# theEricMa/ScaleDreamer

Hardware: AMD Instinct MI355X
Metric: ASD train steps/sec (64x64 render, SD2.1) (higher is better)
Workload: dtype f32 renderer / f16 diffusion (f32 accumulate); 1 GPU; asd_sd_nerf: 1 view/GPU, 64x64 rays, 512 spp occgrid march, implicit-volume iNGP (16x2 hash grid 2^19, MLP 64), SD-2.1 UNet batch 5 (CFG+Perp-Neg+shifted t), VAE 512^2 fwd+bwd, AdamW; views_per_gpu=1, parallelism=dp1, diffusion_backend=hip, diffusion_weights=seeded random init (seed 1)

## Files before the change

include/asd_hip.h:

```cpp
#ifndef ASD_HIP_H
#define ASD_HIP_H

#include <stdint.h>

#ifdef __cplusplus
extern "C" {
#endif

#define ASD_MAX_LEVELS 16
#define ASD_OK 0
#define ASD_ERR_ARG 1
#define ASD_ERR_LAUNCH 2
#define ASD_ERR_UNSUPPORTED 3

typedef struct asd_grid_meta {
    uint32_t n_levels;
    uint32_t n_features;
    uint32_t n_params;
    uint32_t reserved;
    float    scale[ASD_MAX_LEVELS];
    uint32_t resolution[ASD_MAX_LEVELS];
    uint32_t offset[ASD_MAX_LEVELS];
    uint32_t size[ASD_MAX_LEVELS];
    uint32_t dense[ASD_MAX_LEVELS];
// ... 252 lines not shown
    int32_t gn_silu;
    int32_t wide_rows;
    int32_t ln_mode;
    float   ln_eps;
    const float* ln_sc;
    float*  ln_stats;
    int32_t a_seg_rows, w_seg_rows;
    int32_t a_seg_off[9], w_seg_off[6];
    int32_t partials_only;
    int32_t gn_apply;
    void*   gn_apply_y;
    const void* gn_apply_gamma; const void* gn_apply_beta;
    float   gn_apply_eps;
    int32_t gn_apply_silu;
    float*  gn_apply_stats;
} asd_gemm_args;
int32_t asd_gemm_gn_records(const asd_gemm_args* args);
int32_t asd_gemm_gn_applies(const asd_gemm_args* args);
int asd_gemm_f16(const asd_gemm_args* args, void* stream);
int asd_gemm_force_tile(int32_t cfg);
enum { ASD_TILE_PLAIN = 0, ASD_TILE_WIN = 1, ASD_TILE_WIN2 = 2, ASD_TILE_PP = 3, ASD_TILE_WS = 4 };
int asd_gemm_tile_info(int32_t i, int32_t* out7);

#define ASD_GN_STATS_FLOATS(batch) (64 * (batch) + 64 * (512 + (batch)))
int asd_groupnorm_f16(const void* x1, int32_t c1, const void* x2, int32_t c2, int32_t batch, int32_t hw,
                      const void* gamma, const void* beta, float eps, int32_t silu, void* y,
                      float* stats ,
                      void* stream);
int asd_groupnorm_ordered_f16(const void* x, int32_t c, int32_t batch, int32_t hw, const void* gamma, const void* beta, float eps,
                              int32_t silu, void* y, float* stats, void* stream);
// ... 280 lines not shown
```

scaledreamer_amd/_lib.py:

```python
from __future__ import annotations

import ctypes as C
import os
from typing import Optional

import torch

_HERE = os.path.dirname(os.path.abspath(__file__))
LIB_PATH = os.environ.get("ASD_HIP_LIB") or os.path.join(_HERE, "libasd_hip.so")
ASD_MAX_LEVELS = 16

ASD_BIAS_CONST, ASD_BIAS_BLOB_MAGIC3D, ASD_BIAS_BLOB_DREAMFUSION, ASD_BIAS_SPHERE = 0, 1, 2, 3
ASD_FIELD_DENSITY, ASD_FIELD_SDF = 0, 1
ASD_ACT_SOFTPLUS, ASD_ACT_EXP, ASD_ACT_TRUNC_EXP, ASD_ACT_NONE = 0, 1, 2, 3


class AsdError(RuntimeError):
    pass


class GridMeta(C.Structure):
    _fields_ = [
        ("n_levels", C.c_uint32),
        ("n_features", C.c_uint32),
# ... 42 lines not shown
        ("lda", C.c_int32), ("ldw", C.c_int32), ("ldc", C.c_int32),
        ("bias", C.c_void_p), ("row_bias", C.c_void_p), ("rows_per_group", C.c_int32),
        ("residual", C.c_void_p), ("ldr", C.c_int32), ("act", C.c_int32), ("out_f32", C.c_int32),
        ("conv", C.c_int32), ("Hin", C.c_int32), ("Win", C.c_int32), ("Cin", C.c_int32), ("Hout", C.c_int32),
        ("Wout", C.c_int32), ("stride", C.c_int32), ("pad", C.c_int32), ("upsample", C.c_int32),
        ("zero_page", C.c_void_p), ("split_k", C.c_int32), ("workspace", C.c_void_p),
        ("tile_cfg", C.c_int32), ("ld_row_bias", C.c_int32), ("group_m", C.c_int32), ("group_n", C.c_int32),
        ("gn_partials", C.c_void_p), ("gn_cg", C.c_int32), ("gn_rows", C.c_int32),
        ("gn_bwd_x", C.c_void_p), ("gn_bwd_fstats", C.c_void_p), ("gn_bwd_gamma", C.c_void_p), ("gn_bwd_beta", C.c_void_p),
        ("gn_eps", C.c_float), ("gn_silu", C.c_int32), ("wide_rows", C.c_int32),
        ("ln_mode", C.c_int32), ("ln_eps", C.c_float), ("ln_sc", C.c_void_p), ("ln_stats", C.c_void_p),
        ("a_seg_rows", C.c_int32), ("w_seg_rows", C.c_int32), ("a_seg_off", C.c_int32 * 9), ("w_seg_off", C.c_int32 * 6),
        ("partials_only", C.c_int32),
        ("gn_apply", C.c_int32), ("gn_apply_y", C.c_void_p), ("gn_apply_gamma", C.c_void_p), ("gn_apply_beta", C.c_void_p),
        ("gn_apply_eps", C.c_float), ("gn_apply_silu", C.c_int32), ("gn_apply_stats", C.c_void_p),
    ]


class RenderParams(C.Structure):
    _fields_ = [("march", MarchCfg), ("meta", C.c_void_p), ("field", C.c_void_p), ("rays_o", C.c_void_p), ("rays_d", C.c_void_p), ("n_rays", C.c_int32),
                ("occ_bits", C.c_void_p), ("jitter", C.c_void_p), ("grid", C.c_void_p), ("w1d", C.c_void_p), ("w2d", C.c_void_p), ("w1f", C.c_void_p),
                ("w2f", C.c_void_p), ("bg", C.c_void_p), ("early_stop_eps", C.c_float), ("alpha_thre", C.c_float), ("prune", C.c_int32),
                ("color_act", C.c_int32), ("capacity", C.c_int32)]


RENDER_LAYOUT_FIELDS = ["total_bytes", "count", "offset", "total", "c_ray_idx", "c_t0", "c_t1", "c_pts", "c_sigma", "keep", "kept", "koff", "n_kept",
                        "ray_idx", "t0", "t1", "pts", "dirs", "sigma", "feats", "enc", "weights", "opacity", "depth", "z_var", "rgb_fg", "comp_rgb",
                        "c_feats", "c_enc"]


# ... 173 lines not shown
```

scaledreamer_amd/csrc/gemm_ws.hip:

```cpp
#include <type_traits>

#include "gemm_tile.h"

typedef float floatx16 __attribute__((ext_vector_type(16)));
typedef unsigned uintx4 __attribute__((ext_vector_type(4)));

#define WS_A_BYTES(NB) ((NB) * 64 * 64)
#define WS_W_BYTES (9 * 64 * 64)
#define WS_PAD 1024
#define WS_LDS_BYTES(NB) (3 * WS_W_BYTES + 2 * WS_A_BYTES(NB) + 2 * WS_PAD)

template <int NB>
__global__ __launch_bounds__(256, 1) void conv3x3_ws_kernel(const asd_gemm_args p) {
    constexpr int A_BYTES = WS_A_BYTES(NB), W_BYTES = WS_W_BYTES;
    constexpr int A_INSTR = A_BYTES / 1024;
    constexpr int A_PER_WAVE = (A_INSTR + 1) / 2;
    extern __shared__ __attribute__((aligned(16))) char smem[];
    char* const w_base = smem;
    char* const a_base = smem + 3 * W_BYTES + WS_PAD;
    const int tid = threadIdx.x, lane = tid & 63, wave = __builtin_amdgcn_readfirstlane(tid >> 6);
    const int wm = wave >> 1, wn = wave & 1;
    const int tiles_n = p.N / 64;
    const int tn = (int)blockIdx.x % tiles_n, kz = (int)blockIdx.x / tiles_n;
    const int n0 = tn * 64;
    const int cs = p.Cin / p.split_k, c0 = kz * cs, n_chunks = cs / 32;
    const bool w_loader = wave < 2;

    const int a_px = lane >> 2;
    const char* a_lane = (const char*)p.A + ((size_t)a_px * p.Cin + c0) * 2;
    const int a_piece_even = ((lane & 3) ^ (a_px >> 3)) * 16, a_piece_odd = ((lane & 3) ^ (2 + (a_px >> 3))) * 16;
    const char* w_lane = (const char*)p.W + ((size_t)(n0 + (lane >> 2)) * p.ldw + c0) * 2 + (((lane & 3) ^ ((lane >> 4) & 3)) * 16);

    auto issue_w = [&](int chunk) {
        char* W_s = w_base + (chunk % 3) * W_BYTES;
#pragma unroll
        for (int j = 0; j < 18; ++j) {
            const int t = wave * 18 + j;
            const size_t off = ((size_t)((t & 3) * 16) * p.ldw + (size_t)(t >> 2) * p.Cin + chunk * 32) * 2;
            __builtin_amdgcn_global_load_lds((const GLOBAL_AS void*)(w_lane + off), (LDS_AS void*)(W_s + t * 1024), 16, 0, 0);
        }
    };
    auto issue_a = [&](int chunk) {
        char* A_s = a_base + (chunk & 1) * A_BYTES;
#pragma unroll
        for (int j = 0; j < A_PER_WAVE; ++j) {
            const int q = (wave - 2) * A_PER_WAVE + j;
            if (q < A_INSTR)
                __builtin_amdgcn_global_load_lds((const GLOBAL_AS void*)(a_lane + ((size_t)q * 16 * p.Cin + chunk * 32) * 2 + ((q & 1) ? a_piece_odd : a_piece_even)),
                                                 (LDS_AS void*)(A_s + q * 1024), 16, 0, 0);
        }
    };

    const int l31 = lane & 31, kh = lane >> 5, yy = l31 >> 3, xx = l31 & 7;
    const unsigned m_x_first = xx == 0 ? 0u : 0xffffffffu, m_x_last = xx == 7 ? 0u : 0xffffffffu;
    const unsigned m_y_first = yy == 0 ? 0u : 0xffffffffu, m_y_last = yy == 3 ? 0u : 0xffffffffu;
    const bool top0 = ((wm * NB) & 1) == 0, top1 = ((wm * NB + 1) & 1) == 0;
    const unsigned m_ky0[2] = {top0 ? m_y_first : 0xffffffffu, top1 ? m_y_first : 0xffffffffu};
    const unsigned m_ky2[2] = {top0 ? 0xffffffffu : m_y_last, top1 ? 0xffffffffu : m_y_last};
    const unsigned a_lane_lds = (unsigned)(size_t)a_base + (unsigned)((wm * NB * 32 + yy * 8 + xx - 9) * 64);
    const unsigned w_lane_lds = (unsigned)(size_t)w_base + (unsigned)((wn * 32 + l31) * 64);
    const int wkey = (l31 >> 2) & 3;
    unsigned a_piece[3][2], w_piece[2];
#pragma unroll
    for (int j = 0; j < 2; ++j) {
        w_piece[j] = (unsigned)(((2 * j + kh) ^ wkey) * 16);
#pragma unroll
        for (int ky = 0; ky < 3; ++ky) a_piece[ky][j] = (unsigned)((((2 * j + kh) ^ ((yy + ky - 1) & 3))) * 16);
    }

    floatx16 acc[NB];
#pragma unroll
    for (int i = 0; i < NB; ++i)
#pragma unroll
        for (int r = 0; r < 16; ++r) acc[i][r] = 0.f;

    struct Frag { uintx4 a[NB]; uintx4 w; };
#define WS_READ16(dst, addr, OFF) asm volatile("ds_read_b128 %0, %1 offset:%2" : "=&v"(dst) : "v"(addr), "n"(OFF) : "memory")

    if (w_loader) {
        issue_w(0);
        if (n_chunks > 1) { issue_w(1); asm volatile("s_waitcnt vmcnt(18)" ::: "memory"); }
        else asm volatile("s_waitcnt vmcnt(0)" ::: "memory");
    } else {
        issue_a(0);
        asm volatile("s_waitcnt vmcnt(0)" ::: "memory");
    }
    __builtin_amdgcn_s_barrier();
    for (int c = 0; c < n_chunks; ++c) {
        if (w_loader) { if (c + 2 < n_chunks) issue_w(c + 2); }
        else if (c + 1 < n_chunks) issue_a(c + 1);
        const unsigned a_slot = a_lane_lds + (unsigned)((c & 1) * A_BYTES), w_slot = w_lane_lds + (unsigned)((c % 3) * W_BYTES);
        unsigned aaddr[3][2], waddr[2];
#pragma unroll
        for (int j = 0; j < 2; ++j) {
            waddr[j] = w_slot + w_piece[j];
#pragma unroll
            for (int ky = 0; ky < 3; ++ky) aaddr[ky][j] = a_slot + a_piece[ky][j];
        }
        auto read_frags = [&](Frag& f, auto step_c) {
            constexpr int step = decltype(step_c)::value, tap = step >> 1, j = step & 1, ky = tap / 3, kx = tap - ky * 3;
            WS_READ16(f.w, waddr[j], tap * 4096);
#define WS_RA(I_) if constexpr (I_ < NB) WS_READ16(f.a[I_], aaddr[ky][j], I_ * 2048 + (8 * ky + kx) * 64)
            WS_RA(0); WS_RA(1); WS_RA(2); WS_RA(3); WS_RA(4);
#undef WS_RA
        };
        auto mma = [&](Frag& f, auto step_c) {
            constexpr int step = decltype(step_c)::value, tap = step >> 1, ky = tap / 3, kx = tap - ky * 3;
            const unsigned mx = kx == 0 ? m_x_first : (kx == 2 ? m_x_last : 0xffffffffu);
            const unsigned m0 = mx & (ky == 0 ? m_ky0[0] : (ky == 2 ? m_ky2[0] : 0xffffffffu));
            const unsigned m1 = mx & (ky == 0 ? m_ky0[1] : (ky == 2 ? m_ky2[1] : 0xffffffffu));
#pragma unroll
            for (int i = 0; i < NB; ++i) {
                if (tap != 4) {
                    const unsigned m = (i & 1) ? m1 : m0;
                    f.a[i][0] &= m; f.a[i][1] &= m; f.a[i][2] &= m; f.a[i][3] &= m;
                }
                acc[i] = __builtin_amdgcn_mfma_f32_32x32x16_f16(__builtin_bit_cast(half8, f.a[i]), __builtin_bit_cast(half8, f.w), acc[i], 0, 0, 0);
            }
        };
        auto wait_frags = [&](Frag& f, auto pending_c) {
            constexpr int pending = decltype(pending_c)::value;
            if constexpr (NB == 5) asm volatile("s_waitcnt lgkmcnt(%6)" : "+v"(f.a[0]), "+v"(f.a[1]), "+v"(f.a[2]), "+v"(f.a[3]), "+v"(f.a[4]), "+v"(f.w) : "n"(pending));
            else if constexpr (NB == 4) asm volatile("s_waitcnt lgkmcnt(%5)" : "+v"(f.a[0]), "+v"(f.a[1]), "+v"(f.a[2]), "+v"(f.a[3]), "+v"(f.w) : "n"(pending));
            else if constexpr (NB == 3) asm volatile("s_waitcnt lgkmcnt(%4)" : "+v"(f.a[0]), "+v"(f.a[1]), "+v"(f.a[2]), "+v"(f.w) : "n"(pending));
            else if constexpr (NB == 2) asm volatile("s_waitcnt lgkmcnt(%3)" : "+v"(f.a[0]), "+v"(f.a[1]), "+v"(f.w) : "n"(pending));
            else asm volatile("s_waitcnt lgkmcnt(%2)" : "+v"(f.a[0]), "+v"(f.w) : "n"(pending));
        };
        Frag f0, f1;
        read_frags(f0, std::integral_constant<int, 0>{});
#define WS_STEP(S_, CUR_, NXT_)                                                                                   \
        if constexpr (S_ + 1 < 18) {                                                                              \
            read_frags(NXT_, std::integral_constant<int, (S_ + 1 < 18 ? S_ + 1 : 17)>{});                          \
            wait_frags(CUR_, std::integral_constant<int, NB + 1>{});                                              \
        } else wait_frags(CUR_, std::integral_constant<int, 0>{});                                                \
        mma(CUR_, std::integral_constant<int, S_>{});                                                             \
        __builtin_amdgcn_sched_barrier(0)
        WS_STEP(0, f0, f1); WS_STEP(1, f1, f0); WS_STEP(2, f0, f1); WS_STEP(3, f1, f0); WS_STEP(4, f0, f1); WS_STEP(5, f1, f0);
        WS_STEP(6, f0, f1); WS_STEP(7, f1, f0); WS_STEP(8, f0, f1); WS_STEP(9, f1, f0); WS_STEP(10, f0, f1); WS_STEP(11, f1, f0);
        WS_STEP(12, f0, f1); WS_STEP(13, f1, f0); WS_STEP(14, f0, f1); WS_STEP(15, f1, f0); WS_STEP(16, f0, f1); WS_STEP(17, f1, f0);
#undef WS_STEP
        if (w_loader && c + 2 < n_chunks) asm volatile("s_waitcnt vmcnt(18)" ::: "memory");
        else asm volatile("s_waitcnt vmcnt(0)" ::: "memory");
        __builtin_amdgcn_s_barrier();
    }
#undef WS_READ16

    float* slab = p.workspace + (size_t)kz * p.M * p.N + n0 + wn * 32 + l31;
#pragma unroll
    for (int i = 0; i < NB; ++i) {
        const int mt = wm * NB + i;
#pragma unroll
        for (int q = 0; q < 4; ++q)
#pragma unroll
            for (int r = 0; r < 4; ++r) {
                const int m = mt * 32 + q * 8 + kh * 4 + r;
                slab[(size_t)m * p.N] = acc[i][q * 4 + r];
            }
    }
}

size_t asd_conv_ws_lds_bytes(int images) { return (size_t)WS_LDS_BYTES(images); }

int asd_conv_ws_launch(const asd_gemm_args* a, hipStream_t s) {
    const int images = a->M / 64;
    const dim3 grid((a->N / 64) * a->split_k);
#define WS_LAUNCH(NB_) asd_launch_lds<conv3x3_ws_kernel<NB_>>(grid, dim3(256), asd_conv_ws_lds_bytes(NB_), s, *a)
    switch (images) {
        case 1: WS_LAUNCH(1); break;
        case 2: WS_LAUNCH(2); break;
        case 3: WS_LAUNCH(3); break;
        case 4: WS_LAUNCH(4); break;
        case 5: WS_LAUNCH(5); break;
        default: return ASD_ERR_ARG;
    }
#undef WS_LAUNCH
    return ASD_OK;
}
```

scaledreamer_amd/csrc/net.hip:

```cpp
#include <cstdlib>
#include <map>
#include <string>
#include <vector>

#include "asd_common.h"

namespace {

typedef _Float16 half_t;

struct WSpec { std::string name; int rows, cols; };

struct Bump {
    char* base = nullptr;
    size_t off = 0, cap = 0;
    void* take(size_t bytes) {
        off = (off + 255) & ~(size_t)255;
        void* p = base ? base + off : nullptr;
        off += bytes;
        return p;
    }
    half_t* halfs(size_t n) { return (half_t*)take(n * 2); }
    float* floats(size_t n) { return (float*)take(n * 4); }
};
// ... 38 lines not shown
        return (int)specs.size() - 1;
    }
    const half_t* w(const std::string& name) const {
        auto it = index.find(name);
        return it == index.end() ? nullptr : (const half_t*)ptr[it->second];
    }
    bool has(const std::string& name) const { return index.count(name) != 0; }
};

int pad32(int c) { return (c + 31) / 32 * 32; }

struct GemmOpt {
    const void* bias = nullptr; const void* row_bias = nullptr; int rows_per_group = 1, ld_row_bias = 0;
    const void* residual = nullptr; int ldr = 0; int act = 0; int out_f32 = 0;
    int gn_rows = 0;
    Act* out = nullptr;
    const half_t* gn_x = nullptr; const float* gn_fstats = nullptr; const half_t* gn_gamma = nullptr; const half_t* gn_beta = nullptr;
    int gn_silu = 0;
    bool gn_bwd_form = false;
    int ln_mode = 0; const float* ln_sc = nullptr; float* ln_stats = nullptr;
    const GnNext* gn_next = nullptr;
};

void set_gn_bwd(asd_gemm_args& g, const GemmOpt& o) {
    g.gn_bwd_x = o.gn_x; g.gn_bwd_fstats = o.gn_fstats; g.gn_bwd_gamma = o.gn_gamma; g.gn_bwd_beta = o.gn_beta;
    g.gn_eps = 1e-6f; g.gn_silu = o.gn_silu;
}

void launch_gemm(Run& r, asd_gemm_args& g, Act* gn_out = nullptr, bool gn_bwd_form = false, const GnNext* gn_next = nullptr) {
    g.zero_page = r.zero_page;
// ... 53 lines not shown
    g.ln_mode = o.ln_mode; g.ln_sc = o.ln_sc; g.ln_stats = o.ln_stats; g.ln_eps = 1e-5f;
    if (o.gn_x) set_gn_bwd(g, o);
    if (o.out) { *o.out = Act{}; o.out->p = (const half_t*)C; }
    launch_gemm(r, g, o.out, o.gn_bwd_form, o.gn_next);
}

void conv3x3(Run& r, const void* x, int B, int Hin, int Win, int Cin, const void* W, int Cout, void* y, int Hout, int Wout, int stride,
             int pad, int upsample, const GemmOpt& o = GemmOpt()) {
    asd_gemm_args g = asd_gemm_args{};
    const int taps = upsample == 3 ? 4 : 9;
    g.A = x; g.W = W; g.C = y; g.M = B * Hout * Wout; g.N = Cout; g.K = taps * Cin; g.lda = 0; g.ldw = taps * Cin; g.ldc = Cout;
    g.bias = o.bias; g.row_bias = o.row_bias; g.rows_per_group = o.row_bias ? o.rows_per_group : 1; g.ld_row_bias = o.ld_row_bias;
    g.residual = o.residual; g.ldr = o.ldr; g.act = o.act; g.out_f32 = o.out_f32;
    g.conv = 1; g.Hin = Hin; g.Win = Win; g.Cin = Cin; g.Hout = Hout; g.Wout = Wout; g.stride = stride; g.pad = pad; g.upsample = upsample;
    g.gn_rows = o.gn_rows;
    if (o.gn_x) set_gn_bwd(g, o);
    if (o.out) { *o.out = Act{}; o.out->p = (const half_t*)y; }
    launch_gemm(r, g, o.out, o.gn_bwd_form, o.gn_next);
}

#define LEAF(call)                                              \
    do {                                                        \
        if (!r.dry && r.status == ASD_OK) {                     \
            const int st__ = (call);                            \
            if (st__ != ASD_OK) r.status = st__;                \
        }                                                       \
    } while (0)

half_t* groupnorm(Run& r, const void* x1, int c1, const void* x2, int c2, int B, int hw, const half_t* gamma, const half_t* beta, float eps,
                  int silu, half_t* y = nullptr, float** stats_out = nullptr, const Act* src = nullptr) {
// ... 14 lines not shown
struct UBlock { std::vector<ULayer> layers; };

struct UNet : Net {
    asd_unet_desc d;
    std::vector<UBlock> inputs, outputs;
    UBlock middle;
    std::map<std::string, int> emb_off, ctx_off;
    int emb_total = 0, ctx_total = 0;
};

#define ASD_LN_FOLD_MIN_C 1024
void u_norm(UNet& n, const std::string& p, int c) { n.add(p + ".weight", 1, c); n.add(p + ".bias", 1, c); }
void u_lin(UNet& n, const std::string& p, int cin, int cout, bool bias = true) { n.add(p + ".weight", cout, cin); if (bias) n.add(p + ".bias", 1, cout); }
void u_conv(UNet& n, const std::string& p, int cin, int cout) { n.add(p + ".weight", cout, 9 * pad32(cin)); n.add(p + ".bias", 1, cout); }

void u_res(UNet& n, const std::string& p, int cin, int cout) {
    u_norm(n, p + ".in_layers.0", cin);
    u_conv(n, p + ".in_layers.2", cin, cout);
    u_norm(n, p + ".out_layers.0", cout);
    u_conv(n, p + ".out_layers.3", cout, cout);
    if (cin != cout) u_lin(n, p + ".skip_connection", cin, cout);
    n.emb_off[p] = n.emb_total;
    n.emb_total += cout;
}
void u_attn(UNet& n, const std::string& p, int c) {
    u_norm(n, p + ".norm", c);
    u_lin(n, p + ".proj_in", c, c);
    for (int dd = 0; dd < n.d.transformer_depth; ++dd) {
        const std::string b = p + ".transformer_blocks." + std::to_string(dd);
        const bool fold = c >= ASD_LN_FOLD_MIN_C;
        if (!fold) for (const char* nm : {".norm1", ".norm2", ".norm3"}) u_norm(n, b + nm, c);
        n.add(b + ".attn1.to_qk.weight", 2 * c, c);
        if (fold) n.add(b + ".attn1.to_qk.ln_sc", 1, 4 * 2 * c);
        n.add(b + ".attn1.to_v.weight", c, c);
        if (fold) n.add(b + ".attn1.to_v.ln_sc", 1, 4 * c);
// ... 13 lines not shown
void unet_build(UNet& n) {
    const asd_unet_desc& d = n.d;
    const int mc = d.model_channels, emb = 4 * mc;
    u_lin(n, "time_embed.0", mc, emb);
    u_lin(n, "time_embed.2", emb, emb);
    if (d.camera_dim > 0) { u_lin(n, "camera_embed.0", d.camera_dim, emb); u_lin(n, "camera_embed.2", emb, emb); }
    u_conv(n, "input_blocks.0.0", d.in_channels, mc);
    n.inputs.push_back(UBlock{{ULayer{0, "input_blocks.0.0", d.in_channels, mc}}});
    std::vector<int> chans{mc};
    int ch = mc, ds = 0;
    for (int lvl = 0; lvl < d.n_levels; ++lvl) {
        const int mult = d.channel_mult[lvl];
        for (int k = 0; k < d.num_res_blocks; ++k) {
            const std::string p = "input_blocks." + std::to_string(n.inputs.size());
            UBlock b;
            u_res(n, p + ".0", ch, mult * mc);
            b.layers.push_back(ULayer{1, p + ".0", ch, mult * mc});
            ch = mult * mc;
            if (d.attention_ds_mask & (1 << ds)) { u_attn(n, p + ".1", ch); b.layers.push_back(ULayer{2, p + ".1", ch, ch}); }
            n.inputs.push_back(b);
            chans.push_back(ch);
        }
        if (lvl != d.n_levels - 1) {
            const std::string p = "input_blocks." + std::to_string(n.inputs.size()) + ".0.op";
            u_conv(n, p, ch, ch);
            n.inputs.push_back(UBlock{{ULayer{3, p, ch, ch}}});
            chans.push_back(ch);
            ++ds;
        }
    }
    u_res(n, "middle_block.0", ch, ch);
    u_attn(n, "middle_block.1", ch);
    u_res(n, "middle_block.2", ch, ch);
    n.middle.layers = {ULayer{1, "middle_block.0", ch, ch}, ULayer{2, "middle_block.1", ch, ch}, ULayer{1, "middle_block.2", ch, ch}};
    for (int lvl = d.n_levels - 1; lvl >= 0; --lvl) {
        const int mult = d.channel_mult[lvl];
        for (int i = 0; i <= d.num_res_blocks; ++i) {
            const int ich = chans.back();
            chans.pop_back();
            const std::string p = "output_blocks." + std::to_string(n.outputs.size());
            UBlock b;
            u_res(n, p + ".0", ch + ich, mc * mult);
            b.layers.push_back(ULayer{1, p + ".0", ch + ich, mc * mult});
            ch = mc * mult;
            int k = 1;
            if (d.attention_ds_mask & (1 << ds)) {
                u_attn(n, p + "." + std::to_string(k), ch);
                b.layers.push_back(ULayer{2, p + "." + std::to_string(k), ch, ch});
                ++k;
            }
            if (lvl && i == d.num_res_blocks) {
                const std::string q = p + "." + std::to_string(k) + ".conv";
                n.add(q + ".weight", 4 * ch, 4 * pad32(ch)); n.add(q + ".bias", 1, ch);
                b.layers.push_back(ULayer{4, q, ch, ch});
                --ds;
            }
            n.outputs.push_back(b);
// ... 21 lines not shown
    return dst;
}

Act u_resblock(UNet& n, Run& r, const UState& s, const std::string& p, const Act& xin, int cin, int cout, int Hh, int Ww, const GnNext* next = nullptr) {
    const int B = s.B, hw = Hh * Ww, M = B * hw;
    const half_t* x = xin.p;
    half_t* t1 = groupnorm(r, x, cin, nullptr, 0, B, hw, n.w(p + ".in_layers.0.weight"), n.w(p + ".in_layers.0.bias"), 1e-5f, 1, nullptr, nullptr, &xin);
    half_t* t2 = r.mem.halfs((size_t)M * cout);
    Act a2;
    GemmOpt o1;
    o1.bias = n.w(p + ".in_layers.2.bias");
    o1.row_bias = s.emb_all + n.emb_off[p]; o1.rows_per_group = hw; o1.ld_row_bias = s.emb_ld;
    o1.gn_rows = hw; o1.out = &a2;
    const GnNext gn2{n.w(p + ".out_layers.0.weight"), n.w(p + ".out_layers.0.bias"), 1e-5f, 1};
    o1.gn_next = &gn2;
    conv3x3(r, t1, B, Hh, Ww, cin, n.w(p + ".in_layers.2.weight"), cout, t2, Hh, Ww, 1, 1, 0, o1);
    half_t* t3 = groupnorm(r, t2, cout, nullptr, 0, B, hw, n.w(p + ".out_layers.0.weight"), n.w(p + ".out_layers.0.bias"), 1e-5f, 1, nullptr, nullptr, &a2);
    const half_t* skip = x;
    if (n.has(p + ".skip_connection.weight")) {
        half_t* sk = r.mem.halfs((size_t)M * cout);
        GemmOpt os;
        os.bias = n.w(p + ".skip_connection.bias");
        gemm(r, x, M, cin, n.w(p + ".skip_connection.weight"), cout, cin, cin, sk, cout, os);
        skip = sk;
    }
    half_t* out = r.mem.halfs((size_t)M * cout);
    Act ao;
    GemmOpt o2;
    o2.bias = n.w(p + ".out_layers.3.bias"); o2.residual = skip; o2.ldr = cout; o2.gn_rows = hw; o2.out = &ao; o2.gn_next = next;
    conv3x3(r, t3, B, Hh, Ww, cout, n.w(p + ".out_layers.3.weight"), cout, out, Hh, Ww, 1, 1, 0, o2);
    return ao;
}

half_t* layernorm(Run& r, const half_t* x, int rows, int c, const half_t* g, const half_t* b) {
    half_t* y = r.mem.halfs((size_t)rows * c);
    LEAF(asd_layernorm_f16(x, rows, c, g, b, 1e-5f, y, r.stream));
    return y;
}

Act u_transformer(UNet& n, Run& r, const UState& s_in, const std::string& p, const Act& xin, int C, int Hh, int Ww, const GnNext* next = nullptr) {
    const UState* sp = &s_in;
    int B = sp->B, L = Hh * Ww, M = B * L;
    const int heads = C / 64, F = sp->F;
    const half_t* x = xin.p;
// ... 862 lines not shown
```

scaledreamer_amd/diffusion/hip_ops.py:

```python
from __future__ import annotations

import ctypes as C
import os
from typing import Optional

import torch

from .. import _lib as L
from .._lib import GemmArgs, check, f32, i32, lib, ptr, stream

_zero = {}
_gn_stats = {}


def zero_page(device) -> torch.Tensor:
    key = str(device)
    if key not in _zero:
        _zero[key] = torch.zeros(256, dtype=torch.uint8, device=device)
    return _zero[key]


def _p(t: Optional[torch.Tensor]):
    return None if t is None else C.c_void_p(t.data_ptr())

# ... 79 lines not shown
        _tune_scratch[key] = torch.empty(TUNE_SCRATCH_BYTES, dtype=torch.uint8, device=device)
    return _tune_scratch[key]


def release_tune_scratch() -> None:
    _tune_scratch.clear()


if os.environ.get("ASD_GEMM_PLAN_FILE", "") != "none" and os.path.exists(L.LIB_PATH):
    load_plans()


def gemm(a: torch.Tensor, w: torch.Tensor, bias=None, row_bias=None, rows_per_group: int = 0, residual=None, act: int = 0,
         out: Optional[torch.Tensor] = None, out_f32: bool = False, split_k: Optional[int] = None, conv: Optional[dict] = None,
         M: Optional[int] = None, tile_cfg: int = 0, gn_rows: int = 0, gn_bwd: Optional[dict] = None, ln: Optional[dict] = None,
         gn_apply: Optional[dict] = None):
    dev = a.device
    N, K = w.shape
    if conv is not None and int(conv.get("upsample", 0)) == 3:
        N //= 4
    if conv is None:
        assert a.stride(-1) == 1 and a.dim() == 2
        M = a.shape[0]
        lda = a.stride(0)
    else:
        lda = 0
    if out is None:
        out = torch.empty((M, N // 2 if act == 2 else N), device=dev, dtype=torch.float32 if out_f32 else torch.float16)
    g = GemmArgs()
    g.A, g.W, g.C = a.data_ptr(), w.data_ptr(), out.data_ptr()
    g.M, g.N, g.K = M, N, K
# ... 1 lines not shown
    g.bias = None if bias is None else bias.data_ptr()
    g.row_bias = None if row_bias is None else row_bias.data_ptr()
    if row_bias is not None:
        assert row_bias.stride(-1) == 1 and row_bias.shape[-1] == N, "row_bias: [groups, N] with unit column stride"
        g.ld_row_bias = row_bias.stride(0) if row_bias.dim() == 2 and row_bias.shape[0] > 1 else N
    g.rows_per_group = rows_per_group if row_bias is not None else 1
    g.residual = None if residual is None else residual.data_ptr()
    g.ldr = 0 if residual is None else residual.stride(0)
    g.act, g.out_f32 = act, int(out_f32)
    if conv is not None:
        g.conv = 1
        for k in ("Hin", "Win", "Cin", "Hout", "Wout", "stride", "pad", "upsample"):
            setattr(g, k, int(conv[k]))
    g.zero_page = zero_page(dev).data_ptr()
    g.tile_cfg = tile_cfg
    if ln is not None:
        g.ln_mode, g.ln_eps, g.ln_sc = int(ln["mode"]), float(ln.get("eps", 1e-5)), ln["sc"].data_ptr()
        g.ln_stats = None if ln.get("stats") is None else ln["stats"].data_ptr()
    if split_k is not None:
        g.split_k = split_k
    else:
        g.split_k = 0
        if AUTOTUNE and plan_of(g) is None and not torch.cuda.is_current_stream_capturing():
            sc = tune_scratch(dev)
            check(lib().asd_gemm_tune(C.byref(g), C.c_void_p(sc.data_ptr()), C.c_int64(sc.numel()), stream()))
    need = lib().asd_gemm_workspace_bytes(C.byref(g))
    ws = None
    if need > 0:
        ws = torch.empty(need, device=dev, dtype=torch.uint8)
        g.workspace = ws.data_ptr()
# ... 44 lines not shown
    return y.view(B, Ho, Wo, cout)


def pack_upsample_conv3x3_weight(w: torch.Tensor) -> torch.Tensor:
    from .weights import _pack_upsample_conv3x3

    return _pack_upsample_conv3x3(w).contiguous()


def pack_conv3x3_weight(w: torch.Tensor, cin_pad: Optional[int] = None) -> torch.Tensor:
    from .weights import _pack_conv3x3

    return _pack_conv3x3(w, cin_pad).contiguous()


def groupnorm(x1: torch.Tensor, gamma, beta, eps: float, silu: bool, x2: Optional[torch.Tensor] = None,
              return_stats: bool = False):
    B = x1.shape[0]
    c1 = x1.shape[-1]
    c2 = 0 if x2 is None else x2.shape[-1]
    hw = x1.numel() // (B * c1)
    y = torch.empty(tuple(x1.shape[:-1]) + (c1 + c2,), device=x1.device, dtype=torch.float16)
    stats = torch.empty(B * 64 + (512 + B) * 64, device=x1.device, dtype=torch.float32)
    check(lib().asd_groupnorm_f16(ptr(x1), i32(c1), _p(x2), i32(c2), i32(B), i32(hw), ptr(gamma), ptr(beta), f32(eps),
                                  i32(int(silu)), ptr(y), ptr(stats), stream()))
    return (y, stats[:B * 64]) if return_stats else y


def groupnorm_apply(x: torch.Tensor, gamma, beta, eps: float, silu: bool, records: torch.Tensor):
    B, c = x.shape[0], x.shape[-1]
# ... 105 lines not shown
```

scaledreamer_amd/diffusion/weights.py:

```python
from __future__ import annotations

import zlib
from dataclasses import dataclass, field
from typing import Dict, List, Optional, Tuple

import torch


@dataclass
class UNetConfig:
    in_channels: int = 4
    out_channels: int = 4
    model_channels: int = 320
    attention_resolutions: Tuple[int, ...] = (4, 2, 1)
    num_res_blocks: int = 2
    channel_mult: Tuple[int, ...] = (1, 2, 4, 4)
    num_head_channels: int = 64
    transformer_depth: int = 1
    context_dim: int = 1024
    camera_dim: Optional[int] = None

    @property
    def time_embed_dim(self) -> int:
        return self.model_channels * 4
# ... 227 lines not shown
        n = 1
        for d in shp:
            n *= d
        total += n
    return total


def _pack_conv3x3(w: torch.Tensor, cin_pad: Optional[int] = None) -> torch.Tensor:
    cout, cin = w.shape[:2]
    cp = cin_pad or ((cin + 31) // 32 * 32)
    wp = torch.zeros((cout, 3, 3, cp), dtype=w.dtype, device=w.device)
    wp[..., :cin] = w.permute(0, 2, 3, 1)
    return wp.reshape(cout, 9 * cp)


def _pack_upsample_conv3x3(w: torch.Tensor) -> torch.Tensor:
    cout, cin = w.shape[:2]
    cp = (cin + 31) // 32 * 32
    taps = {0: ((0,), (1, 2)), 1: ((0, 1), (2,))}
    wf = w.float()
    out = torch.zeros((2, 2, cout, 2, 2, cp), dtype=torch.float32, device=w.device)
    for a in (0, 1):
        for b in (0, 1):
            for dy in (0, 1):
                for dx in (0, 1):
                    acc = 0
                    for ky in taps[a][dy]:
                        for kx in taps[b][dx]:
                            acc = acc + wf[:, :, ky, kx]
                    out[a, b, :, dy, dx, :cin] = acc
# ... 18 lines not shown
def pack_unet(p: Dict[str, torch.Tensor], cfg: UNetConfig) -> Dict[str, torch.Tensor]:
    _, inputs, middle, outputs = unet_layout(cfg)
    out: Dict[str, torch.Tensor] = {}
    emb_w, emb_b, ck, cv = [], [], [], []
    up_convs = {n + ".weight" for blk in outputs for kind, n, _, _ in blk.layers if kind == "up"}
    for name, t in p.items():
        if ".emb_layers.1." in name or any(k in name for k in (".attn1.to_q.", ".attn1.to_k.", ".attn2.to_k.", ".attn2.to_v.")):
            continue
        if name.endswith(".weight") and t.ndim == 4:
            if name in up_convs:
                out[name] = _pack_upsample_conv3x3(t)
            else:
                out[name] = _pack_conv3x3(t) if t.shape[-1] == 3 else t.reshape(t.shape[0], t.shape[1])
        else:
            out[name] = t
    for blk in list(inputs) + [middle] + list(outputs):
        for kind, name, cin, cout in blk.layers:
            if kind == "res":
                emb_w.append(p[name + ".emb_layers.1.weight"])
                emb_b.append(p[name + ".emb_layers.1.bias"])
            elif kind == "attn":
                for d in range(cfg.transformer_depth):
                    b = f"{name}.transformer_blocks.{d}"
                    ck.append(p[b + ".attn2.to_k.weight"])
                    cv.append(p[b + ".attn2.to_v.weight"])
                    perm = _geglu_rows(4 * cout).to(p[b + ".ff.net.0.proj.weight"].device)
                    out[b + ".ff.net.0.proj.bias"] = p[b + ".ff.net.0.proj.bias"][perm]
                    if cout < LN_FOLD_MIN_C:
                        out[b + ".attn1.to_qk.weight"] = torch.cat([p[b + ".attn1.to_q.weight"], p[b + ".attn1.to_k.weight"]], 0)
                        out[b + ".ff.net.0.proj.weight"] = p[b + ".ff.net.0.proj.weight"][perm]
# ... 110 lines not shown
```

Measured before the change: 73.31 steps/s.

## Stream conv3x3 WS weights directly to registers with pre-tiled weight layout

The weight-stationary 3x3 conv kernel no longer stages weights through LDS with dedicated loader waves. Every wave now loads its own weight fragments from global memory straight into VGPR/AGPR register buffers, triple-buffered across chunks, while the activation tile uses a 4-deep LDS ring loaded by all waves. A new pre-tiled weight copy (W_ws) for the deepest UNet level gives coalesced contiguous per-lane loads. This frees LDS bandwidth and removes the loader/consumer wave split, at the cost of much higher register pressure, extra weight memory, and hand-tuned vmcnt accounting.

```diff
diff --git a/include/asd_hip.h b/include/asd_hip.h
--- a/include/asd_hip.h
+++ b/include/asd_hip.h
@@ -290,6 +290,7 @@
     float   gn_apply_eps;
     int32_t gn_apply_silu;
     float*  gn_apply_stats;
+    const void* W_ws;
 } asd_gemm_args;
 int32_t asd_gemm_gn_records(const asd_gemm_args* args);
 int32_t asd_gemm_gn_applies(const asd_gemm_args* args);
diff --git a/scaledreamer_amd/_lib.py b/scaledreamer_amd/_lib.py
--- a/scaledreamer_amd/_lib.py
+++ b/scaledreamer_amd/_lib.py
@@ -80,6 +80,7 @@
         ("partials_only", C.c_int32),
         ("gn_apply", C.c_int32), ("gn_apply_y", C.c_void_p), ("gn_apply_gamma", C.c_void_p), ("gn_apply_beta", C.c_void_p),
         ("gn_apply_eps", C.c_float), ("gn_apply_silu", C.c_int32), ("gn_apply_stats", C.c_void_p),
+        ("W_ws", C.c_void_p),
     ]
 
 
diff --git a/scaledreamer_amd/csrc/gemm_ws.hip b/scaledreamer_amd/csrc/gemm_ws.hip
--- a/scaledreamer_amd/csrc/gemm_ws.hip
+++ b/scaledreamer_amd/csrc/gemm_ws.hip
@@ -6,67 +6,68 @@
 typedef unsigned uintx4 __attribute__((ext_vector_type(4)));
 
 #define WS_A_BYTES(NB) ((NB) * 64 * 64)
-#define WS_W_BYTES (9 * 64 * 64)
+#define WS_W_TILE_BYTES (9 * 64 * 64)
 #define WS_PAD 1024
-#define WS_LDS_BYTES(NB) (3 * WS_W_BYTES + 2 * WS_A_BYTES(NB) + 2 * WS_PAD)
+#define WS_LDS_BYTES(NB) (4 * WS_A_BYTES(NB) + 2 * WS_PAD)
 
-template <int NB>
+template <int NB, bool TILED>
 __global__ __launch_bounds__(256, 1) void conv3x3_ws_kernel(const asd_gemm_args p) {
-    constexpr int A_BYTES = WS_A_BYTES(NB), W_BYTES = WS_W_BYTES;
-    constexpr int A_INSTR = A_BYTES / 1024;
-    constexpr int A_PER_WAVE = (A_INSTR + 1) / 2;
+    constexpr int A_BYTES = WS_A_BYTES(NB);
+    constexpr int BATCH = 18 + NB;
+    static_assert(2 * BATCH < 64, "vmcnt is a 6-bit counter");
     extern __shared__ __attribute__((aligned(16))) char smem[];
-    char* const w_base = smem;
-    char* const a_base = smem + 3 * W_BYTES + WS_PAD;
+    char* const a_base = smem + WS_PAD;
     const int tid = threadIdx.x, lane = tid & 63, wave = __builtin_amdgcn_readfirstlane(tid >> 6);
     const int wm = wave >> 1, wn = wave & 1;
     const int tiles_n = p.N / 64;
     const int tn = (int)blockIdx.x % tiles_n, kz = (int)blockIdx.x / tiles_n;
     const int n0 = tn * 64;
     const int cs = p.Cin / p.split_k, c0 = kz * cs, n_chunks = cs / 32;
-    const bool w_loader = wave < 2;
+    const int l31 = lane & 31, kh = lane >> 5, yy = l31 >> 3, xx = l31 & 7;
 
     const int a_px = lane >> 2;
     const char* a_lane = (const char*)p.A + ((size_t)a_px * p.Cin + c0) * 2;
     const int a_piece_even = ((lane & 3) ^ (a_px >> 3)) * 16, a_piece_odd = ((lane & 3) ^ (2 + (a_px >> 3))) * 16;
-    const char* w_lane = (const char*)p.W + ((size_t)(n0 + (lane >> 2)) * p.ldw + c0) * 2 + (((lane & 3) ^ ((lane >> 4) & 3)) * 16);
-
-    auto issue_w = [&](int chunk) {
-        char* W_s = w_base + (chunk % 3) * W_BYTES;
+    auto issue_a = [&](int chunk) {
+        char* A_s = a_base + (chunk & 3) * A_BYTES;
 #pragma unroll
-        for (int j = 0; j < 18; ++j) {
-            const int t = wave * 18 + j;
-            const size_t off = ((size_t)((t & 3) * 16) * p.ldw + (size_t)(t >> 2) * p.Cin + chunk * 32) * 2;
-            __builtin_amdgcn_global_load_lds((const GLOBAL_AS void*)(w_lane + off), (LDS_AS void*)(W_s + t * 1024), 16, 0, 0);
+        for (int j = 0; j < NB; ++j) {
+            const int q = wave * NB + j;
+            __builtin_amdgcn_global_load_lds((const GLOBAL_AS void*)(a_lane + ((size_t)q * 16 * p.Cin + chunk * 32) * 2 + ((q & 1) ? a_piece_odd : a_piece_even)),
+                                             (LDS_AS void*)(A_s + q * 1024), 16, 0, 0);
         }
     };
-    auto issue_a = [&](int chunk) {
-        char* A_s = a_base + (chunk & 1) * A_BYTES;
-#pragma unroll
-        for (int j = 0; j < A_PER_WAVE; ++j) {
-            const int q = (wave - 2) * A_PER_WAVE + j;
-            if (q < A_INSTR)
-                __builtin_amdgcn_global_load_lds((const GLOBAL_AS void*)(a_lane + ((size_t)q * 16 * p.Cin + chunk * 32) * 2 + ((q & 1) ? a_piece_odd : a_piece_even)),
-                                                 (LDS_AS void*)(A_s + q * 1024), 16, 0, 0);
-        }
+    const char* w_slice;
+    unsigned w_lane_off;
+    if constexpr (TILED) {
+        w_slice = (const char*)p.W_ws + ((size_t)tn * (p.Cin / 32) + c0 / 32) * WS_W_TILE_BYTES + wn * 2048;
+        w_lane_off = (unsigned)lane * 16u;
+    } else {
+        w_slice = (const char*)p.W + ((size_t)n0 * p.ldw + c0) * 2;
+        w_lane_off = (unsigned)(wn * 32 + l31) * (unsigned)p.ldw * 2u + (unsigned)kh * 16u;
+    }
+    uintx4 wr[3][18];
+    auto load_w = [&](auto r_c, auto fresh_c, int chunk, auto step_c) {
+        constexpr int R = decltype(r_c)::value, step = decltype(step_c)::value, tap = step >> 1, j = step & 1, off = TILED ? j * 1024 : j * 32;
+        constexpr bool fresh = decltype(fresh_c)::value;
+        const char* b = TILED ? w_slice + (size_t)chunk * WS_W_TILE_BYTES + tap * 4096 : w_slice + ((size_t)tap * p.Cin + chunk * 32) * 2;
+#define WS_GLOAD(C_) asm volatile("global_load_dwordx4 %0, %1, %2 offset:%3" : C_(wr[R][step]) : "v"(w_lane_off), "s"(b), "n"(off) : "memory")
+        if constexpr (R == 2) { if constexpr (fresh) WS_GLOAD("=&a"); else WS_GLOAD("+a"); }
+        else { if constexpr (fresh) WS_GLOAD("=&v"); else WS_GLOAD("+v"); }
+#undef WS_GLOAD
     };
 
-    const int l31 = lane & 31, kh = lane >> 5, yy = l31 >> 3, xx = l31 & 7;
     const unsigned m_x_first = xx == 0 ? 0u : 0xffffffffu, m_x_last = xx == 7 ? 0u : 0xffffffffu;
     const unsigned m_y_first = yy == 0 ? 0u : 0xffffffffu, m_y_last = yy == 3 ? 0u : 0xffffffffu;
     const bool top0 = ((wm * NB) & 1) == 0, top1 = ((wm * NB + 1) & 1) == 0;
     const unsigned m_ky0[2] = {top0 ? m_y_first : 0xffffffffu, top1 ? m_y_first : 0xffffffffu};
     const unsigned m_ky2[2] = {top0 ? 0xffffffffu : m_y_last, top1 ? 0xffffffffu : m_y_last};
     const unsigned a_lane_lds = (unsigned)(size_t)a_base + (unsigned)((wm * NB * 32 + yy * 8 + xx - 9) * 64);
-    const unsigned w_lane_lds = (unsigned)(size_t)w_base + (unsigned)((wn * 32 + l31) * 64);
-    const int wkey = (l31 >> 2) & 3;
-    unsigned a_piece[3][2], w_piece[2];
+    unsigned a_piece[3][2];
 #pragma unroll
-    for (int j = 0; j < 2; ++j) {
-        w_piece[j] = (unsigned)(((2 * j + kh) ^ wkey) * 16);
+    for (int j = 0; j < 2; ++j)
 #pragma unroll
         for (int ky = 0; ky < 3; ++ky) a_piece[ky][j] = (unsigned)((((2 * j + kh) ^ ((yy + ky - 1) & 3))) * 16);
-    }
 
     floatx16 acc[NB];
 #pragma unroll
@@ -74,32 +75,33 @@
 #pragma unroll
         for (int r = 0; r < 16; ++r) acc[i][r] = 0.f;
 
-    struct Frag { uintx4 a[NB]; uintx4 w; };
+    struct Frag { uintx4 a[NB]; };
 #define WS_READ16(dst, addr, OFF) asm volatile("ds_read_b128 %0, %1 offset:%2" : "=&v"(dst) : "v"(addr), "n"(OFF) : "memory")
+    auto wait_chunk = [&](int next, int newest) {
+        const int last = n_chunks - 1, young = (newest < last ? newest : last) - next;
+        if (young >= 2) asm volatile("s_waitcnt vmcnt(%0)" ::"n"(2 * BATCH) : "memory");
+        else if (young == 1) asm volatile("s_waitcnt vmcnt(%0)" ::"n"(BATCH) : "memory");
+        else asm volatile("s_waitcnt vmcnt(0)" ::: "memory");
+    };
+    auto issue_batch = [&](auto r_c, int chunk) __attribute__((always_inline)) {
+#define WS_L(S_) load_w(r_c, std::true_type{}, chunk, std::integral_constant<int, S_>{})
+        WS_L(0); WS_L(1); WS_L(2); WS_L(3); WS_L(4); WS_L(5); WS_L(6); WS_L(7); WS_L(8); WS_L(9); WS_L(10); WS_L(11); WS_L(12); WS_L(13); WS_L(14); WS_L(15); WS_L(16); WS_L(17);
+#undef WS_L
+        issue_a(chunk);
+        __builtin_amdgcn_sched_barrier(0);
+    };
 
-    if (w_loader) {
-        issue_w(0);
-        if (n_chunks > 1) { issue_w(1); asm volatile("s_waitcnt vmcnt(18)" ::: "memory"); }
-        else asm volatile("s_waitcnt vmcnt(0)" ::: "memory");
-    } else {
-        issue_a(0);
-        asm volatile("s_waitcnt vmcnt(0)" ::: "memory");
-    }
-    __builtin_amdgcn_s_barrier();
-    for (int c = 0; c < n_chunks; ++c) {
-        if (w_loader) { if (c + 2 < n_chunks) issue_w(c + 2); }
-        else if (c + 1 < n_chunks) issue_a(c + 1);
-        const unsigned a_slot = a_lane_lds + (unsigned)((c & 1) * A_BYTES), w_slot = w_lane_lds + (unsigned)((c % 3) * W_BYTES);
-        unsigned aaddr[3][2], waddr[2];
+    auto chunk = [&](auto r_c, int c) __attribute__((always_inline)) {
+        constexpr int R = decltype(r_c)::value;
+        const bool refill = c + 3 < n_chunks;
+        const unsigned a_slot = a_lane_lds + (unsigned)((c & 3) * A_BYTES);
+        unsigned aaddr[3][2];
 #pragma unroll
-        for (int j = 0; j < 2; ++j) {
-            waddr[j] = w_slot + w_piece[j];
+        for (int j = 0; j < 2; ++j)
 #pragma unroll
             for (int ky = 0; ky < 3; ++ky) aaddr[ky][j] = a_slot + a_piece[ky][j];
-        }
         auto read_frags = [&](Frag& f, auto step_c) {
             constexpr int step = decltype(step_c)::value, tap = step >> 1, j = step & 1, ky = tap / 3, kx = tap - ky * 3;
-            WS_READ16(f.w, waddr[j], tap * 4096);
 #define WS_RA(I_) if constexpr (I_ < NB) WS_READ16(f.a[I_], aaddr[ky][j], I_ * 2048 + (8 * ky + kx) * 64)
             WS_RA(0); WS_RA(1); WS_RA(2); WS_RA(3); WS_RA(4);
 #undef WS_RA
@@ -115,33 +117,47 @@
                     const unsigned m = (i & 1) ? m1 : m0;
                     f.a[i][0] &= m; f.a[i][1] &= m; f.a[i][2] &= m; f.a[i][3] &= m;
                 }
-                acc[i] = __builtin_amdgcn_mfma_f32_32x32x16_f16(__builtin_bit_cast(half8, f.a[i]), __builtin_bit_cast(half8, f.w), acc[i], 0, 0, 0);
+                acc[i] = __builtin_amdgcn_mfma_f32_32x32x16_f16(__builtin_bit_cast(half8, f.a[i]), __builtin_bit_cast(half8, wr[R][step]), acc[i], 0, 0, 0);
             }
         };
         auto wait_frags = [&](Frag& f, auto pending_c) {
             constexpr int pending = decltype(pending_c)::value;
-            if constexpr (NB == 5) asm volatile("s_waitcnt lgkmcnt(%6)" : "+v"(f.a[0]), "+v"(f.a[1]), "+v"(f.a[2]), "+v"(f.a[3]), "+v"(f.a[4]), "+v"(f.w) : "n"(pending));
-            else if constexpr (NB == 4) asm volatile("s_waitcnt lgkmcnt(%5)" : "+v"(f.a[0]), "+v"(f.a[1]), "+v"(f.a[2]), "+v"(f.a[3]), "+v"(f.w) : "n"(pending));
-            else if constexpr (NB == 3) asm volatile("s_waitcnt lgkmcnt(%4)" : "+v"(f.a[0]), "+v"(f.a[1]), "+v"(f.a[2]), "+v"(f.w) : "n"(pending));
-            else if constexpr (NB == 2) asm volatile("s_waitcnt lgkmcnt(%3)" : "+v"(f.a[0]), "+v"(f.a[1]), "+v"(f.w) : "n"(pending));
-            else asm volatile("s_waitcnt lgkmcnt(%2)" : "+v"(f.a[0]), "+v"(f.w) : "n"(pending));
+            if constexpr (NB == 5) asm volatile("s_waitcnt lgkmcnt(%5)" : "+v"(f.a[0]), "+v"(f.a[1]), "+v"(f.a[2]), "+v"(f.a[3]), "+v"(f.a[4]) : "n"(pending));
+            else if constexpr (NB == 4) asm volatile("s_waitcnt lgkmcnt(%4)" : "+v"(f.a[0]), "+v"(f.a[1]), "+v"(f.a[2]), "+v"(f.a[3]) : "n"(pending));
+            else if constexpr (NB == 3) asm volatile("s_waitcnt lgkmcnt(%3)" : "+v"(f.a[0]), "+v"(f.a[1]), "+v"(f.a[2]) : "n"(pending));
+            else if constexpr (NB == 2) asm volatile("s_waitcnt lgkmcnt(%2)" : "+v"(f.a[0]), "+v"(f.a[1]) : "n"(pending));
+            else asm volatile("s_waitcnt lgkmcnt(%1)" : "+v"(f.a[0]) : "n"(pending));
         };
         Frag f0, f1;
         read_frags(f0, std::integral_constant<int, 0>{});
 #define WS_STEP(S_, CUR_, NXT_)                                                                                   \
         if constexpr (S_ + 1 < 18) {                                                                              \
             read_frags(NXT_, std::integral_constant<int, (S_ + 1 < 18 ? S_ + 1 : 17)>{});                          \
-            wait_frags(CUR_, std::integral_constant<int, NB + 1>{});                                              \
+            wait_frags(CUR_, std::integral_constant<int, NB>{});                                                  \
         } else wait_frags(CUR_, std::integral_constant<int, 0>{});                                                \
         mma(CUR_, std::integral_constant<int, S_>{});                                                             \
+        if (refill) load_w(r_c, std::false_type{}, c + 3, std::integral_constant<int, S_>{});                     \
         __builtin_amdgcn_sched_barrier(0)
         WS_STEP(0, f0, f1); WS_STEP(1, f1, f0); WS_STEP(2, f0, f1); WS_STEP(3, f1, f0); WS_STEP(4, f0, f1); WS_STEP(5, f1, f0);
         WS_STEP(6, f0, f1); WS_STEP(7, f1, f0); WS_STEP(8, f0, f1); WS_STEP(9, f1, f0); WS_STEP(10, f0, f1); WS_STEP(11, f1, f0);
         WS_STEP(12, f0, f1); WS_STEP(13, f1, f0); WS_STEP(14, f0, f1); WS_STEP(15, f1, f0); WS_STEP(16, f0, f1); WS_STEP(17, f1, f0);
 #undef WS_STEP
-        if (w_loader && c + 2 < n_chunks) asm volatile("s_waitcnt vmcnt(18)" ::: "memory");
-        else asm volatile("s_waitcnt vmcnt(0)" ::: "memory");
-        __builtin_amdgcn_s_barrier();
+        if (refill) { issue_a(c + 3); __builtin_amdgcn_sched_barrier(0); }
+        if (c + 1 < n_chunks) {
+            wait_chunk(c + 1, c + 3);
+            __builtin_amdgcn_s_barrier();
+        }
+    };
+
+    issue_batch(std::integral_constant<int, 0>{}, 0);
+    if (n_chunks > 1) issue_batch(std::integral_constant<int, 1>{}, 1);
+    if (n_chunks > 2) issue_batch(std::integral_constant<int, 2>{}, 2);
+    wait_chunk(0, 2);
+    __builtin_amdgcn_s_barrier();
+    for (int c = 0; c < n_chunks; c += 3) {
+        chunk(std::integral_constant<int, 0>{}, c);
+        if (c + 1 < n_chunks) chunk(std::integral_constant<int, 1>{}, c + 1);
+        if (c + 2 < n_chunks) chunk(std::integral_constant<int, 2>{}, c + 2);
     }
 #undef WS_READ16
 
@@ -164,7 +180,9 @@
 int asd_conv_ws_launch(const asd_gemm_args* a, hipStream_t s) {
     const int images = a->M / 64;
     const dim3 grid((a->N / 64) * a->split_k);
-#define WS_LAUNCH(NB_) asd_launch_lds<conv3x3_ws_kernel<NB_>>(grid, dim3(256), asd_conv_ws_lds_bytes(NB_), s, *a)
+#define WS_LAUNCH(NB_)                                                                                                         \
+    if (a->W_ws) asd_launch_lds<conv3x3_ws_kernel<NB_, true>>(grid, dim3(256), asd_conv_ws_lds_bytes(NB_), s, *a);            \
+    else asd_launch_lds<conv3x3_ws_kernel<NB_, false>>(grid, dim3(256), asd_conv_ws_lds_bytes(NB_), s, *a)
     switch (images) {
         case 1: WS_LAUNCH(1); break;
         case 2: WS_LAUNCH(2); break;
diff --git a/scaledreamer_amd/csrc/net.hip b/scaledreamer_amd/csrc/net.hip
--- a/scaledreamer_amd/csrc/net.hip
+++ b/scaledreamer_amd/csrc/net.hip
@@ -76,6 +76,7 @@
     const void* bias = nullptr; const void* row_bias = nullptr; int rows_per_group = 1, ld_row_bias = 0;
     const void* residual = nullptr; int ldr = 0; int act = 0; int out_f32 = 0;
     int gn_rows = 0;
+    const void* w_ws = nullptr;
     Act* out = nullptr;
     const half_t* gn_x = nullptr; const float* gn_fstats = nullptr; const half_t* gn_gamma = nullptr; const half_t* gn_beta = nullptr;
     int gn_silu = 0;
@@ -159,6 +160,7 @@
     g.residual = o.residual; g.ldr = o.ldr; g.act = o.act; g.out_f32 = o.out_f32;
     g.conv = 1; g.Hin = Hin; g.Win = Win; g.Cin = Cin; g.Hout = Hout; g.Wout = Wout; g.stride = stride; g.pad = pad; g.upsample = upsample;
     g.gn_rows = o.gn_rows;
+    g.W_ws = o.w_ws;
     if (o.gn_x) set_gn_bwd(g, o);
     if (o.out) { *o.out = Act{}; o.out->p = (const half_t*)y; }
     launch_gemm(r, g, o.out, o.gn_bwd_form, o.gn_next);
@@ -203,11 +205,15 @@
 void u_lin(UNet& n, const std::string& p, int cin, int cout, bool bias = true) { n.add(p + ".weight", cout, cin); if (bias) n.add(p + ".bias", 1, cout); }
 void u_conv(UNet& n, const std::string& p, int cin, int cout) { n.add(p + ".weight", cout, 9 * pad32(cin)); n.add(p + ".bias", 1, cout); }
 
-void u_res(UNet& n, const std::string& p, int cin, int cout) {
+void u_res(UNet& n, const std::string& p, int cin, int cout, bool deepest = false) {
     u_norm(n, p + ".in_layers.0", cin);
     u_conv(n, p + ".in_layers.2", cin, cout);
     u_norm(n, p + ".out_layers.0", cout);
     u_conv(n, p + ".out_layers.3", cout, cout);
+    if (deepest && cin % 32 == 0 && cout % 64 == 0) {
+        n.add(p + ".in_layers.2.weight_ws", cout, 9 * cin);
+        n.add(p + ".out_layers.3.weight_ws", cout, 9 * cout);
+    }
     if (cin != cout) u_lin(n, p + ".skip_connection", cin, cout);
     n.emb_off[p] = n.emb_total;
     n.emb_total += cout;
@@ -251,7 +257,7 @@
         for (int k = 0; k < d.num_res_blocks; ++k) {
             const std::string p = "input_blocks." + std::to_string(n.inputs.size());
             UBlock b;
-            u_res(n, p + ".0", ch, mult * mc);
+            u_res(n, p + ".0", ch, mult * mc, lvl == d.n_levels - 1);
             b.layers.push_back(ULayer{1, p + ".0", ch, mult * mc});
             ch = mult * mc;
             if (d.attention_ds_mask & (1 << ds)) { u_attn(n, p + ".1", ch); b.layers.push_back(ULayer{2, p + ".1", ch, ch}); }
@@ -266,9 +272,9 @@
             ++ds;
         }
     }
-    u_res(n, "middle_block.0", ch, ch);
+    u_res(n, "middle_block.0", ch, ch, true);
     u_attn(n, "middle_block.1", ch);
-    u_res(n, "middle_block.2", ch, ch);
+    u_res(n, "middle_block.2", ch, ch, true);
     n.middle.layers = {ULayer{1, "middle_block.0", ch, ch}, ULayer{2, "middle_block.1", ch, ch}, ULayer{1, "middle_block.2", ch, ch}};
     for (int lvl = d.n_levels - 1; lvl >= 0; --lvl) {
         const int mult = d.channel_mult[lvl];
@@ -277,7 +283,7 @@
             chans.pop_back();
             const std::string p = "output_blocks." + std::to_string(n.outputs.size());
             UBlock b;
-            u_res(n, p + ".0", ch + ich, mc * mult);
+            u_res(n, p + ".0", ch + ich, mc * mult, lvl == d.n_levels - 1);
             b.layers.push_back(ULayer{1, p + ".0", ch + ich, mc * mult});
             ch = mc * mult;
             int k = 1;
@@ -329,6 +335,7 @@
     o1.gn_rows = hw; o1.out = &a2;
     const GnNext gn2{n.w(p + ".out_layers.0.weight"), n.w(p + ".out_layers.0.bias"), 1e-5f, 1};
     o1.gn_next = &gn2;
+    o1.w_ws = n.w(p + ".in_layers.2.weight_ws");
     conv3x3(r, t1, B, Hh, Ww, cin, n.w(p + ".in_layers.2.weight"), cout, t2, Hh, Ww, 1, 1, 0, o1);
     half_t* t3 = groupnorm(r, t2, cout, nullptr, 0, B, hw, n.w(p + ".out_layers.0.weight"), n.w(p + ".out_layers.0.bias"), 1e-5f, 1, nullptr, nullptr, &a2);
     const half_t* skip = x;
@@ -343,6 +350,7 @@
     Act ao;
     GemmOpt o2;
     o2.bias = n.w(p + ".out_layers.3.bias"); o2.residual = skip; o2.ldr = cout; o2.gn_rows = hw; o2.out = &ao; o2.gn_next = next;
+    o2.w_ws = n.w(p + ".out_layers.3.weight_ws");
     conv3x3(r, t3, B, Hh, Ww, cout, n.w(p + ".out_layers.3.weight"), cout, out, Hh, Ww, 1, 1, 0, o2);
     return ao;
 }
diff --git a/scaledreamer_amd/diffusion/hip_ops.py b/scaledreamer_amd/diffusion/hip_ops.py
--- a/scaledreamer_amd/diffusion/hip_ops.py
+++ b/scaledreamer_amd/diffusion/hip_ops.py
@@ -117,7 +117,7 @@
 def gemm(a: torch.Tensor, w: torch.Tensor, bias=None, row_bias=None, rows_per_group: int = 0, residual=None, act: int = 0,
          out: Optional[torch.Tensor] = None, out_f32: bool = False, split_k: Optional[int] = None, conv: Optional[dict] = None,
          M: Optional[int] = None, tile_cfg: int = 0, gn_rows: int = 0, gn_bwd: Optional[dict] = None, ln: Optional[dict] = None,
-         gn_apply: Optional[dict] = None):
+         gn_apply: Optional[dict] = None, w_ws: Optional[torch.Tensor] = None):
     dev = a.device
     N, K = w.shape
     if conv is not None and int(conv.get("upsample", 0)) == 3:
@@ -149,6 +149,9 @@
             setattr(g, k, int(conv[k]))
     g.zero_page = zero_page(dev).data_ptr()
     g.tile_cfg = tile_cfg
+    if w_ws is not None:
+        assert w_ws.is_contiguous() and w_ws.numel() == w.numel() and w_ws.dtype == w.dtype
+        g.W_ws = w_ws.data_ptr()
     if ln is not None:
         g.ln_mode, g.ln_eps, g.ln_sc = int(ln["mode"]), float(ln.get("eps", 1e-5)), ln["sc"].data_ptr()
         g.ln_stats = None if ln.get("stats") is None else ln["stats"].data_ptr()
@@ -223,6 +226,12 @@
     return _pack_conv3x3(w, cin_pad).contiguous()
 
 
+def pack_conv3x3_ws_weight(w_packed: torch.Tensor) -> torch.Tensor:
+    from .weights import pack_conv3x3_ws
+
+    return pack_conv3x3_ws(w_packed).contiguous()
+
+
 def groupnorm(x1: torch.Tensor, gamma, beta, eps: float, silu: bool, x2: Optional[torch.Tensor] = None,
               return_stats: bool = False):
     B = x1.shape[0]
diff --git a/scaledreamer_amd/diffusion/weights.py b/scaledreamer_amd/diffusion/weights.py
--- a/scaledreamer_amd/diffusion/weights.py
+++ b/scaledreamer_amd/diffusion/weights.py
@@ -265,6 +265,14 @@
     return wp.reshape(cout, 9 * cp)
 
 
+def pack_conv3x3_ws(wp: torch.Tensor) -> torch.Tensor:
+    cout, k = wp.shape
+    cin = k // 9
+    assert k == 9 * cin and cout % 64 == 0 and cin % 32 == 0, (cout, k)
+    v = wp.reshape(cout // 64, 2, 32, 9, cin // 32, 2, 2, 8)
+    return v.permute(0, 4, 3, 1, 5, 6, 2, 7).reshape(cout, k)
+
+
 def _pack_upsample_conv3x3(w: torch.Tensor) -> torch.Tensor:
     cout, cin = w.shape[:2]
     cp = (cin + 31) // 32 * 32
@@ -313,6 +321,21 @@
                 out[name] = _pack_conv3x3(t) if t.shape[-1] == 3 else t.reshape(t.shape[0], t.shape[1])
         else:
             out[name] = t
+    deepest, level, last = [layer[1] for layer in middle.layers if layer[0] == "res"], 0, len(cfg.channel_mult) - 1
+    for blk in inputs:
+        for kind, name, _, _ in blk.layers:
+            level += kind == "down"
+            if kind == "res" and level == last:
+                deepest.append(name)
+    for blk in outputs:
+        for kind, name, _, _ in blk.layers:
+            if kind == "res" and level == last:
+                deepest.append(name)
+            level -= kind == "up"
+    for name in deepest:
+        w1, w2 = out[name + ".in_layers.2.weight"], out[name + ".out_layers.3.weight"]
+        if (w1.shape[1] // 9) % 32 == 0 and w1.shape[0] % 64 == 0:
+            out[name + ".in_layers.2.weight_ws"], out[name + ".out_layers.3.weight_ws"] = pack_conv3x3_ws(w1), pack_conv3x3_ws(w2)
     for blk in list(inputs) + [middle] + list(outputs):
         for kind, name, cin, cout in blk.layers:
             if kind == "res":
```

Result: no change. 73.55 steps/s, median of 6 (+0.3%).
